# SudeepDasari/visual_foresight

Measured on AMD Instinct MI355X. Metric: predicted frames/sec (whole node), 200-sample x 13-step x 64x64 CEM, higher is better.
Workload: dtype f32

## Files before the change

### visual_foresight_amd/csrc/vf_conv_first.h

```cpp
#pragma once
#include <hip/hip_runtime.h>
#include "vf_conv_mfma.h"

namespace vf {

constexpr int kFirstK = 5, kFirstStride = 2, kFirstCin = 3;
__host__ __device__ constexpr int first_patch_stride(const int TW) { return (((TW - 1) * kFirstStride + kFirstK) * kFirstCin + 1) & ~1; }
__host__ __device__ constexpr size_t first_lds_floats(const int TH, const int TW) {
    return (size_t)((TH - 1) * kFirstStride + kFirstK) * first_patch_stride(TW) + 32;
}

template <int CO, class PT>
__device__ __forceinline__ void conv_first_tile(const PT &p, const int bx_, float *smem) {
    static_assert(CO % 4 == 0 && CO <= 32, "first conv: 4 - 32 output channels");
    typedef const __attribute__((address_space(4))) float cfloat;
    const int bx = __builtin_amdgcn_readfirstlane(bx_);
    const int tid = threadIdx.x, lane = tid & 63, wave = tid >> 6;
    const int tiles_per_img = p.tilesY * p.tilesX;
    const int b = bx / tiles_per_img, tile_id = bx - b * tiles_per_img;
    const int ty0 = (tile_id / p.tilesX) * p.TH, tx0 = (tile_id % p.tilesX) * p.TW;
    const int PH = (p.TH - 1) * kFirstStride + kFirstK, PW3 = ((p.TW - 1) * kFirstStride + kFirstK) * kFirstCin;
    const int PS = first_patch_stride(p.TW);
    float *s_in = smem;
    long long *red = reinterpret_cast<long long *>(smem + (size_t)PH * PS);
// ... 88 lines not shown
            else __builtin_amdgcn_raw_buffer_store_b128(__builtin_bit_cast(u32x4_, v), r_out, o, 0, 0);
        }
        const long long wsum = wave_sum(ssum), wsq = wave_sum(ssq);
        if (lane == 0) { red[2 * wave] = wsum; red[2 * wave + 1] = wsq; }
        __syncthreads();
        if (tid == 0) {
            long long su = 0, sq = 0;
            for (int w = 0; w < 4; ++w) { su += red[2 * w]; sq += red[2 * w + 1]; }
            long long *dst = p.stats + ((long long)b * p.stats_nparts + tile_id) * 2;
            if (wt) {
                __hip_atomic_store(dst, su, __ATOMIC_RELAXED, __HIP_MEMORY_SCOPE_AGENT);
                __hip_atomic_store(dst + 1, sq, __ATOMIC_RELAXED, __HIP_MEMORY_SCOPE_AGENT);
            } else {
                dst[0] = su; dst[1] = sq;
            }
        }
    }
}

template <int CO>
VF_GLOBAL VF_LAUNCH_BOUNDS(kConvThreads, 2) void conv_first_kernel(const ConvParams p) {
    extern __shared__ __attribute__((aligned(16))) float smem[];
    conv_first_tile<CO>(p, blockIdx.x, smem);
}

}
```

### visual_foresight_amd/csrc/vf_conv_mfma.h

```cpp
#pragma once
#include <hip/hip_runtime.h>
#include <type_traits>

#ifdef VF_HOST_SELFTEST
#define VF_GLOBAL __device__
#define VF_LAUNCH_BOUNDS(...)
#else
#define VF_GLOBAL __global__
#define VF_LAUNCH_BOUNDS(...) __launch_bounds__(__VA_ARGS__)
#endif

namespace vf {

constexpr int kPollSleep = 16;

#ifdef VF_TILE_STATS
__device__ unsigned long long g_tile_clk[32][8];
#define VF_TS_NOW() (threadIdx.x == 0 ? wall_clock64() : 0ull)
#define VF_TS_ADD(KEY_, SLOT_, DT_) do { if (threadIdx.x == 0) atomicAdd(&g_tile_clk[KEY_][SLOT_], (unsigned long long)(DT_)); } while (0)
#else
#define VF_TS_NOW() 0ull
#define VF_TS_ADD(KEY_, SLOT_, DT_) do { } while (0)
#endif

// ... 63 lines not shown
__host__ __device__ constexpr int fused_epi(int nd, bool first, bool k6 = false) {
    return EPI_CONVT_FUSED + 2 * (nd - 1) + (first ? 1 : 0) + (k6 ? 8 : 0);
}
__host__ __device__ constexpr int fused_epi_flow(int nd) { return EPI_CONVT_FUSED + 16 + 2 * (nd - 1); }
__host__ __device__ constexpr int fused_epi_dna(int nd) { return fused_epi_flow(nd) + 1; }
static_assert(fused_epi_dna(4) < EPI_CONV_PAIR, "the fused epilogues end in front of EPI_CONV_PAIR");

struct ConvSeg {
    const float *ptr;
    long long bstride;
    int C;
    int nchunk;
    const long long *ln_part;
    long long ln_bstride;
    int ln_nparts;
    float ln_inv_n;
    const float *gamma;
    const float *beta;
    int gamma_mod;
    int relu;
};

struct ConvParams {
    ConvSeg seg[2];
    int nseg;
    int B;
    int Hin, Win;
    int Hout, Wout;
    int KH, KW, stride, pad;
    int KC;
    int NI, TH, TW, RPI;
    int tilesY, tilesX;
    int ncg;
    int Cout;
    const float *Wp;
    const unsigned short *Wp16;
    const float *bias;
    const float *sbias;
    int sbias_ld;
    float *out;
    float *cstate;
    const float *cstate_in;
    long long cin_bstride;
    long long *stats;
    int stats_nparts;
    int chunks_per_split;
    int n_valid;
    int tile_variant;
    const void *fuse_comp;
    const void *fuse_next;
    int *fuse_ready;
    const int *fuse_status;
    int fuse_view, fuse_nd;
    const int *late_cnt;
    int late_expect, late_mode;
    int *late_status;
    int *cu_state;
    int yield_budget;
    int wt_out;
    const float *cond_bias;
// ... 120 lines not shown
        s += __builtin_trunc(d * kStatScale);
        q += __builtin_trunc(d * d * kStatScale);
    }
    __device__ __forceinline__ long long sum() const { return (long long)s; }
    __device__ __forceinline__ long long sumsq() const { return (long long)q; }
};
__device__ __forceinline__ void ln_from_totals(const long long su, const long long sq, const float inv_n,
                                               float &mean, float &rstd) {
    const double m = (double)su * (1.0 / kStatScale) * (double)inv_n;
    double var = (double)sq * (1.0 / kStatScale) * (double)inv_n - m * m;
    var = var < 0.0 ? 0.0 : var;
    mean = (float)m;
    rstd = (float)(1.0 / sqrt(var + (double)kLnEps));
}

struct TileDiv {
    unsigned magic; int d;
    __device__ __forceinline__ explicit TileDiv(const int d_) : magic(0xFFFFFFFFu / (unsigned)d_ + 1u), d(d_) {}
    __device__ __forceinline__ int div(const int n) const { return d == 1 ? n : (int)__umulhi((unsigned)n, magic); }
};

template <class PT>
__device__ __forceinline__ void ln_table(const PT &p, const int bimg0, float *lnTab, const int s_begin = 0,
                                         const int s_end = 2) {
    const int tid = threadIdx.x, lane = tid & 63, wave = tid >> 6;
    const int n = min(s_end, p.nseg) * p.NI, i0 = s_begin * p.NI;
    if (p.nseg * p.NI <= 8) {
        for (int i = i0 + wave; i < n; i += kConvThreads / 64) {
            const int s = i / p.NI, img = i - s * p.NI;
            const auto &sg = p.seg[s];
            float mean = 0.f, rstd = 1.f;
            const int b = bimg0 + img;
            if (sg.ln_part && b < p.B) {
                long long su = 0, sq = 0;
                const long long *pp = sg.ln_part + (long long)b * sg.ln_bstride;
                for (int k = lane; k < sg.ln_nparts; k += 64) { su += pp[2 * k]; sq += pp[2 * k + 1]; }
                su = wave_sum(su); sq = wave_sum(sq);
                ln_from_totals(su, sq, sg.ln_inv_n, mean, rstd);
            }
            if (lane == 0) { lnTab[2 * i] = mean; lnTab[2 * i + 1] = rstd; }
        }
    } else {
        for (int i = i0 + tid; i < n; i += kConvThreads) {
            const int s = i / p.NI, img = i % p.NI;
            const auto &sg = p.seg[s];
            float mean = 0.f, rstd = 1.f;
            const int b = bimg0 + img;
            if (sg.ln_part && b < p.B) {
                long long su = 0, sq = 0;
                const long long *pp = sg.ln_part + (long long)b * sg.ln_bstride;
                for (int k = 0; k < sg.ln_nparts; ++k) { su += pp[2 * k]; sq += pp[2 * k + 1]; }
                ln_from_totals(su, sq, sg.ln_inv_n, mean, rstd);
            }
            lnTab[2 * i] = mean;
            lnTab[2 * i + 1] = rstd;
        }
    }
}

__device__ __forceinline__ void lstm_cell(const float gi, const float gj, const float gf, const float go,
                                          const float c_old, float &c_new, float &h_new) {
    c_new = fmaf(c_old, sigmoidf_(gf + 1.0f), sigmoidf_(gi) * tanhf_(gj));
    h_new = tanhf_(c_new) * sigmoidf_(go);
}

struct LstmRowAddr {
// ... 214 lines not shown
        if (lane == 0) { red[2 * wave] = wsum; red[2 * wave + 1] = wsq; }
        __syncthreads();
        auto put = [&](long long *dst, const long long su, const long long sq) {
            if (p.wt_out != 0) {
                __hip_atomic_store(dst, su, __ATOMIC_RELAXED, __HIP_MEMORY_SCOPE_AGENT);
                __hip_atomic_store(dst + 1, sq, __ATOMIC_RELAXED, __HIP_MEMORY_SCOPE_AGENT);
            } else {
                dst[0] = su; dst[1] = sq;
            }
        };
        if (p.NI == 1) {
            if (tid == 0 && bimg0 < p.B) {
                long long su = 0, sq = 0;
                for (int w = 0; w < 4; ++w) { su += red[2 * w]; sq += red[2 * w + 1]; }
                put(p.stats + ((long long)bimg0 * p.stats_nparts + tile_id * p.ncg + cg) * 2, su, sq);
            }
        } else {
            const int waves_per_img = p.RPI / WROWS;
            if (lane == 0 && (wave % waves_per_img) == 0) {
                const int img = wave / waves_per_img;
                const int b = bimg0 + img;
                if (img < p.NI && b < p.B) {
                    long long su = 0, sq = 0;
                    for (int w = 0; w < waves_per_img; ++w) { su += red[2 * (wave + w)]; sq += red[2 * (wave + w) + 1]; }
                    put(p.stats + ((long long)b * p.stats_nparts + cg) * 2, su, sq);
                }
            }
        }
    }
}

template <class F, int... I>
__device__ __forceinline__ void static_for_impl(F &&f, std::integer_sequence<int, I...>) {
    (f(std::integral_constant<int, I>{}), ...);
}
template <int N, class F>
__device__ __forceinline__ void static_for(F &&f) { static_for_impl(f, std::make_integer_sequence<int, N>{}); }

template <int MR, class PT>
__device__ __forceinline__ void gs_acc_init(const PT &p, f32x16 (&acc)[MR][1], const int cg, const int ty0, const int tx0) {
// ... 158 lines not shown
        for (int img = 0; img < p.NI; ++img) {
            if (bimg0 + img >= p.B) continue;
            long long su = 0, sq = 0;
            for (int w = 0; w < 4; ++w) {
                const int wrb = MR < 4 ? (w & (MR - 1)) : w;
                if (p.NI == 1 || (wrb * 32) / p.RPI == img) { su += red[2 * w]; sq += red[2 * w + 1]; }
            }
            long long *dst = p.stats + ((long long)(bimg0 + img) * p.stats_nparts +
                                        (p.NI == 1 ? tile_id * p.ncg + cg : cg)) * 2;
            if (wt) {
                __hip_atomic_store(dst, su, __ATOMIC_RELAXED, __HIP_MEMORY_SCOPE_AGENT);
                __hip_atomic_store(dst + 1, sq, __ATOMIC_RELAXED, __HIP_MEMORY_SCOPE_AGENT);
            } else {
                dst[0] = su; dst[1] = sq;
            }
        }
    }
}

template <int MR, class PT>
__device__ __forceinline__ void gates_raw_epilogue(const PT &p, f32x16 (&acc)[MR][1], const int bx, const int by, float *smem) {
    static_assert(MR == 4, "raw gate epilogue: 128-row tile");
    const int tid = threadIdx.x, lane = tid & 63, wave = tid >> 6;
    const int cg = by;
    const int tiles_per_img = p.tilesY * p.tilesX;
    int bimg0, ty0, tx0;
    if (p.NI == 1) {
        bimg0 = bx / tiles_per_img;
        const int tile_id = bx % tiles_per_img;
        ty0 = (tile_id / p.tilesX) * p.TH;
// ... 813 lines not shown
```

### visual_foresight_amd/csrc/vf_engine.hip

```cpp
#include <hip/hip_runtime.h>

#include <algorithm>
#include <cmath>
#include <cstdio>
#include <cstring>
#include <cstdlib>
#include <string>
#include <type_traits>
#include <vector>

#include <dlfcn.h>
#ifdef VF_HOST_SELFTEST
#include <sys/mman.h>
#endif

#include "../../include/vf_hip.h"
#include "vf_conv_mfma.h"
#include "vf_small_kernels.h"
#include "vf_goal_image.h"
#include "vf_frame_scorer.h"
#include "vf_registration_net.h"
#include "vf_inverse_model.h"
#include "vf_plan_render.h"
#include "vf_resize.h"
// ... 492 lines not shown
    } sched[2];
    int last_sched = 0;
    size_t sched_capacity = 0, counter_capacity = 0;
    PhaseDesc *stage[kSchedRing] = {nullptr};
    hipEvent_t stage_done[kSchedRing] = {nullptr};
    bool stage_used[kSchedRing] = {false};
    int stage_next = 0;
    int *d_sync = nullptr;
    int xcd_queues = kQueues;
    bool early_start = true;
    bool fuse_top = true;
    bool fuse_pair = true;
    bool wt_publish = VF_WT_DEFAULT != 0;
    bool pad_skip = true;
    bool share_recurrent = true;
    int yield_budget = -1;
    bool pair_allowed = true;
    int *d_status = nullptr;
    unsigned long long *d_stats = nullptr;
    bool phase_stats = false;
    int persist_wgs_per_cu = 2;
    size_t max_lds = 0;

    bool cache_shared = true, shared_valid = false;
    int shared_cfg = -1;

    bool profiling = false;
    std::vector<hipEvent_t> ev_pool;
    size_t ev_used = 0;
    double prof_flops = 0.0;
// ... 432 lines not shown
    }
    VF_ALLOC(h->ctx_states, (size_t)nc * c.sdim);
    VF_ALLOC(h->ctx_actions, (size_t)std::max(nc - 1, 1) * c.adim);

    row_spec(h, h->base.frames_all, (size_t)T * H * W * 3, false);
    if (ND > 0) row_spec(h, h->base.distrib_all, (size_t)T * H * W * ND, false);
    row_spec(h, h->base.states_all, (size_t)T * c.sdim, false);
    if ((rc = alloc_view(h, h->base, (size_t)Bc * NV, false))) return rc;
    h->frames_all = h->base.frames_all; h->distrib_all = h->base.distrib_all; h->states_all = h->base.states_all;
    h->sums_view_stride = (long long)Bc * ND * h->nblocks * 2;
    h->sums_step_stride = h->sums_view_stride * NV;
    if (ND > 0) VF_ALLOC(h->sums, (size_t)T * h->sums_step_stride);
    VF_ALLOC(h->goal_mse, (size_t)Bc * NV * T);
    VF_ALLOC(h->actions_buf, (size_t)Bc * T * c.adim);
    h->sched_capacity = ((size_t)h->S * phases_per_step + 8) * NV;
    h->counter_capacity = h->sched_capacity * ((size_t)Bc + 1);
    VF_ALLOC(h->sched[0].d_phases, h->sched_capacity);
    VF_ALLOC(h->sched[1].d_phases, h->sched_capacity);
    VF_ALLOC(h->d_sync, kSyncHead + h->counter_capacity);
    VF_ALLOC(h->d_status, 1);
    VF_ALLOC(h->d_stats, h->sched_capacity * 2);
    return VF_OK;
}

#define VF_EMIT(var, expr)                 \
    const int var = (expr);                \
    if (Sink::failed(var)) return var;

#include "vf_engine_savp3.inc"

extern "C" {

int vf_abi_version(void) { return VF_ABI_VERSION; }

// ... 210 lines not shown
int vf_create(const vf_config *cfg, vf_handle **out) {
    vf_handle *made = nullptr;
    VF_API_TRY
    if (!out) return fail(VF_ERR_INVALID, "null out pointer");
    *out = nullptr;
    int rc = validate(cfg);
    if (rc) return rc;
#ifndef VF_HOST_SELFTEST
    VF_HIP_CHECK(hipSetDevice(cfg->device));
#endif
    vf_handle *h = new vf_handle();
    made = h;
    h->cfg = *cfg;
    if (const char *e = getenv("VF_PAD_SKIP")) h->pad_skip = atoi(e) != 0;
    if (const char *e = getenv("VF_SHARE_RECURRENT")) h->share_recurrent = atoi(e) != 0;
    h->ncam = std::max(1, cfg->ncam);
    h->n_draws = std::max(1, cfg->n_draws);
    h->cfg.ncam = h->ncam; h->cfg.n_draws = h->n_draws;
    h->H = cfg->height; h->W = cfg->width; h->ND = cfg->ndesig; h->K = cfg->num_masks;
    h->T = cfg->sequence_length - cfg->n_context;
    h->S = h->T + cfg->n_context - 1;
    h->table = tensor_table(*cfg);
    h->blob_floats = h->table.back().offset + h->table.back().size();
    h->savp = cfg->arch == 1 || cfg->arch == 2;
    h->cond = cfg->arch == 2;
    h->flow = is_flow(*cfg);
    h->dna = is_dna(*cfg);
    h->stp = is_stp(*cfg);
    h->Hc = h->savp ? h->H / 2 : h->H; h->Wc = h->savp ? h->W / 2 : h->W;
    const int H = h->H, W = h->W;
// ... 345 lines not shown
            int , int dfin, bool ) {
        int rc = conv(PH_CONVT_RAW, l, p, {});
        if (rc) return rc;
        return composite(cp, ntiles, view, {dfin});
    }
    static bool failed(int rc) { return rc != VF_OK; }
};
#endif

struct ScheduleSink {
    std::vector<PhaseDesc> phases;
    int next_ticket = 0, next_counter = 0;
    double flops = 0.0;
    size_t max_lds = 0;

    static PhaseDep dep_on(const PhaseDesc &Q) {
        PhaseDep dp;
        dp.cnt_base = Q.cnt_base;
        if (Q.whole) { dp.mode = 1; dp.expect = Q.n_items; }
        else {
            dp.mode = (Q.B == 1) ? 1 : 0;
            switch (Q.type) {
                case PH_SA: case PH_CDNA_FIN: case PH_COND: case PH_STP_FIN: dp.expect = 1; break;
                case PH_COMPOSITE: dp.expect = Q.gx; break;
                case PH_EW: dp.expect = Q.ew.spi > 0 ? 1 : Q.gx; break;
                default: dp.expect = (Q.NI == 1 ? Q.tiles_per_img : 1) * Q.gy;
            }
        }
        return dp;
    }
// ... 34 lines not shown
        P.ew = p; P.view = view;
        P.gx = p.spi > 0 ? 1 : p.gx; P.gy = 1;
        max_lds = std::max(max_lds, ew_lds_bytes(p.op, p.op == EW_TOP3 ? p.top.ND : 1));
        return add(P, ew_items(p), p.B, deps);
    }
    int conv_late(int type, const ConvLayer &l, const ConvParams &p, int u_early, int u_late, int u_extra = -1) {
        PhaseDep ld;
        if (!late_dep(u_late, ld)) return conv(type, l, p, {u_early, u_late, u_extra});
        const int u = conv(type, l, p, {u_early, u_extra});
        if (u >= 0) { phases[u].has_late = 1; phases[u].late = ld; }
        return u;
    }
    int conv(int type, const ConvLayer &l, const ConvParams &p, std::initializer_list<int> deps) {
        PhaseDesc P = phase(type, p.B);
        P.conv = p;
        P.NI = l.NI; P.tiles_per_img = l.tilesY * l.tilesX;
        P.gx = conv_items_x(l, p.B);
        P.gy = l.ncg;
        if (l.tile == TILE_FC_WIDE) P.gy = 1;
        P.whole = type == PH_FC_PARTIAL;
        P.tile = l.tile; P.mrep = l.mrep;
        P.prec = p.tile_variant;
        max_lds = std::max(max_lds, l.lds_bytes);
        flops += conv_flops(type, l, p);
        return add(P, P.gx * P.gy * l.nsplit, P.whole ? 1 : p.B, deps);
    }
    int sa(const SaParams &p, std::initializer_list<int> deps) {
        PhaseDesc P = phase(PH_SA, p.B);
        P.sa = p;
        return add(P, (p.B + kSaPerItem - 1) / kSaPerItem, p.B, deps);
    }
    static bool pair_capable() { return true; }
    static const ConvLayer &fc_plan(const vf_handle *h) { return h->fc_wide_ok ? h->fc_wide : h->fc; }
    static bool pairable(const ConvLayer &a, const ConvLayer &b) {
        return a.mode == PACK_PLAIN && b.mode == PACK_PLAIN && a.nseg == 1 && b.nseg == 1 && a.ncg == 2 && b.ncg == 2 &&
               a.Cout == 64 && b.segC[0] == 64 && b.Cout <= 64 && b.KH == 1 && b.KW == 1 && b.stride == 1 && b.pad == 0 &&
               b.KC == 32 && a.tilesY * a.tilesX == 1 && b.tilesY * b.tilesX == 1 && a.NI == b.NI && a.RPI == b.RPI &&
               a.TH == b.TH && a.TW == b.TW && a.Hout == b.Hout && a.Wout == b.Wout && a.nsplit == 1 && b.nsplit == 1 &&
               (a.KH * a.KW * (a.KC / 8)) % 2 == 0 &&
               a.lds_bytes >= (size_t)2 * 128 * 36 * 4;
    }
    int conv_pair(const ConvLayer &a, const ConvParams &pa, const ConvLayer &b, const ConvParams &pb,
                  std::initializer_list<int> deps) {
        PhaseDesc P = phase(PH_CONV_PAIR, pa.B);
        P.conv = pa; P.conv2 = pb;
        P.conv.ncg = 1;
        P.NI = a.NI; P.tiles_per_img = 1;
        P.gx = (pa.B + a.NI - 1) / a.NI; P.gy = 1;
        P.mrep = 1;
        max_lds = std::max(max_lds, a.lds_bytes);
        const double rows = (double)pa.B * a.Hout * a.Wout;
        flops += 2.0 * rows * a.KH * a.KW * a.segC[0] * a.Cout + 2.0 * rows * b.segC[0] * b.Cout;
        return add(P, P.gx, pa.B, deps);
    }
    int fin(const FinParams &p, std::initializer_list<int> deps) {
        PhaseDesc P = phase(PH_CDNA_FIN, p.B);
        P.fin = p;
        return add(P, p.B, p.B, deps);
    }
    int stp_fin(const StpFinParams &p, std::initializer_list<int> deps) {
// ... 5 lines not shown
    int composite(const CompositeParams &p, int ntiles, int view, std::initializer_list<int> deps) {
        PhaseDesc P = phase(PH_COMPOSITE, p.B);
        P.comp = p; P.gx = ntiles; P.view = view;
        return add(P, ntiles * p.B, p.B, deps);
    }
    static bool fusable(const ConvLayer &l, int ND) { return top_fusable(l, ND); }
    int top(const ConvLayer &l, const ConvParams &p, const CompositeParams &cp, int ntiles, int view, int d_early,
            int d_late, int dfin, bool fuse) {
        if (!fuse || !fusable(l, cp.ND)) {
            const int u = conv_late(PH_CONVT_RAW, l, p, d_early, d_late);
            if (u < 0) return u;
            return composite(cp, ntiles, view, {u, dfin});
        }
        PhaseDesc P = phase(PH_TOP_FUSED, p.B);
        P.conv = p; P.comp = cp; P.view = view;
        P.NI = 1; P.tiles_per_img = l.tilesY * l.tilesX;
        P.gx = p.B * P.tiles_per_img; P.gy = 1;
        P.mrep = 1;
        P.aux_base = next_counter + p.B;
        max_lds = std::max(max_lds, std::max(l.lds_bytes, fused_top_lds_floats(l.TH, l.TW, cp.ND) * 4));
        flops += 2.0 * (double)p.B * l.Hout * l.Wout * 9.0 * (l.segC[0] + (l.nseg > 1 ? l.segC[1] : 0)) * l.Cout;
        if (!late_dep(d_late, P.late)) return add(P, P.gx, 2 * p.B, {d_early, d_late, dfin});
        P.has_late = 1;
        return add(P, P.gx, 2 * p.B, {d_early, dfin});
    }
    static bool failed(int rc) { return rc < 0; }
    static int skipped() { return kSkipped; }
};

template <class Sink>
// ... 316 lines not shown
    int items = 0, counters = 0;
    int nq = 1, total_q[kQueues] = {0};
    double flops = 0.0;
    size_t lds = 0;
};

static int build_schedule(vf_handle *h, int B, bool skip_shared, BuiltSchedule &out) {
    std::vector<ScheduleSink> sinks(h->ncam);
    VF_INJECT(1);
    int counters = 0, rc;
    out.flops = 0.0;
    size_t max_lds = 0;
    for (int v = 0; v < h->ncam; ++v) {
        sinks[v].next_counter = counters;
        sinks[v].early_start = h->early_start;
        if (h->cfg.arch == 3)
            rc = emit_rollout_s3(h, v, B, h->actions_buf, nullptr, sinks[v]);
        else
            rc = emit_rollout(h, v, make_view(h, v, h->actions_buf), h->shared_views[(size_t)v], B, nullptr, sinks[v],
                              skip_shared);
        if (rc < 0) return rc;
        counters = sinks[v].next_counter;
        out.flops += sinks[v].flops;
        max_lds = std::max(max_lds, sinks[v].max_lds);
    }
    out.phases.clear();
    const size_t n = sinks[0].phases.size();
    for (size_t i = 0; i < n; ++i)
        for (int v = 0; v < h->ncam; ++v) out.phases.push_back(sinks[v].phases[i]);
    int ticket = 0;
// ... 114 lines not shown
    for (const AllocRec &a : h->allocs) {
        const char *lo = static_cast<const char *>(a.p);
        if (q >= lo && q + bytes <= lo + a.bytes) return true;
    }
    return false;
}

extern "C" int vf_selftest_schedule(vf_handle *h, int32_t B, int32_t skip_shared, int64_t *out_items,
                                    uint64_t *out_upload_checksum) {
    VF_API_TRY
    if (!h) return fail(VF_ERR_INVALID, "null handle");
    BuiltSchedule bs;
    int rc = build_schedule(h, B, skip_shared != 0, bs);
    if (rc) return rc;
    int ticket = 0;
    for (size_t i = 0; i < bs.phases.size(); ++i) {
        const PhaseDesc &P = bs.phases[i];
        if (P.first_ticket != ticket || P.n_items <= 0) return fail(VF_ERR_INVALID, "tickets are not contiguous");
        ticket += P.n_items;
        if (P.ndep < 0 || P.ndep > kMaxDeps) return fail(VF_ERR_INVALID, "bad dependency count");
        if ((h->flow || h->dna) && (P.type == PH_FC_PARTIAL || P.type == PH_CDNA_FIN))
            return fail(VF_ERR_INVALID, "phase " + std::to_string(i) + ": a CDNA kernel item in " +
                                        (h->dna ? "a DNA schedule" : "an appearance-flow schedule"));
        if (h->stp ? P.type == PH_CDNA_FIN : P.type == PH_STP_FIN)
            return fail(VF_ERR_INVALID, "phase " + std::to_string(i) + (h->stp ? ": a CDNA kernel-finish item (a 5 x 5 kernel table) in an STP schedule"
                                                                              : ": an STP finish item outside an STP schedule"));
        for (int d = 0; d < P.ndep; ++d) {
            bool found = false;
            for (size_t j = 0; j < i && !found; ++j) found = bs.phases[j].cnt_base == P.dep[d].cnt_base;
            if (!found) return fail(VF_ERR_INVALID, "phase " + std::to_string(i) + " depends on a later phase");
// ... 12 lines not shown
            const ConvParams &c2 = P.conv2;
            ok = ok && P.conv.ncg == 1 && c2.ncg == 2 && c2.KC == 32 && c2.nseg == 1 && c2.seg[0].nchunk == 2;
            ok = ok && in_allocs(h, c2.Wp, (size_t)2 * 4 * 2 * 64 * 4 * 4) && in_allocs(h, c2.bias, 64 * 4);
            ok = ok && in_allocs(h, c2.out, (size_t)P.B * c2.Hout * c2.Wout * c2.Cout * 4);
            ok = ok && in_allocs(h, c2.sbias, c2.sbias ? (size_t)((P.B - 1) * c2.sbias_ld + c2.Cout) * 4 : 0);
        }
        if (P.type <= PH_FC_PARTIAL || ph_is_conv(P.type) || P.type == PH_TOP_FUSED || P.type == PH_CONV_PAIR) {
            const ConvParams &c = P.conv;
            for (int s = 0; s < c.nseg; ++s) {
                const long long span = (long long)(P.B - 1) * c.seg[s].bstride + (long long)c.Hin * c.Win * c.seg[s].C;
                ok = ok && in_allocs(h, c.seg[s].ptr, (size_t)span * 4);
                ok = ok && in_allocs(h, c.seg[s].ln_part, c.seg[s].ln_part ? (size_t)((P.B - 1) * c.seg[s].ln_bstride + c.seg[s].ln_nparts * 2) * 8 : 0);
            }
            ok = ok && in_allocs(h, c.Wp, 16) && in_allocs(h, c.bias, 4) && in_allocs(h, c.out, 4);
            ok = ok && in_allocs(h, c.cstate, 4) && in_allocs(h, c.cstate_in, 4) && in_allocs(h, c.stats, 8);
            const size_t gates_bytes = (size_t)c.Hout * c.Wout * 4 * c.Cout * 4;
            if (P.type == PH_GATES_RAW) ok = ok && in_allocs(h, c.out, (size_t)P.B * gates_bytes);
            if (c.chunk_begin != 0)
                ok = ok && (P.type == PH_GATES_RAW ||
                            (P.type == PH_LSTM && (P.tile == TILE_LSTM_GS128 || P.tile == TILE_LSTM_GS64)));
            if (c.acc_init)
                ok = ok && in_allocs(h, c.acc_init, gates_bytes) && P.type == PH_LSTM && P.NI == 1 && !P.has_late &&
                     (P.tile == TILE_LSTM_GS128 || P.tile == TILE_LSTM_GS64) && c.chunk_begin == c.seg[0].nchunk;
        }
        if (P.conv.wt_out != 0) {
            const bool lstm_vec = P.type == PH_LSTM &&
                                  (P.tile == TILE_LSTM_GS128 || P.tile == TILE_LSTM_GS64 || P.tile == TILE_LSTM_ROW32);
            const bool light_vec = P.type >= PH_CONV_RELU && P.type <= PH_CONVT_RAW && P.conv.Cout % 4 == 0 &&
                                   ((P.tile == TILE_CONV && P.mrep == 1) ||
                                    (P.tile == TILE_FIRST_VALU && P.type == PH_CONV_RAW && (P.conv.Cout == 16 || P.conv.Cout == 32)));
// ... 148 lines not shown
                head[q] += P.n_q[q];
                total += P.n_q[q];
            }
            if (bs.nq > 1 && P.q_inner > 1 && ph_is_conv(P.type)) {
                int lo = P.n_q[0], hi = P.n_q[0];
                for (int q = 0; q < bs.nq; ++q) { lo = std::min(lo, P.n_q[q]); hi = std::max(hi, P.n_q[q]); }
                if (hi - lo > 1) return fail(VF_ERR_INVALID, "phase " + std::to_string(i) + ": queues are not balanced");
            }
            for (int q = bs.nq; q < kQueues; ++q)
                if (P.n_q[q]) return fail(VF_ERR_INVALID, "items in an unused queue");
        }
        for (int q = 0; q < bs.nq; ++q)
            if (head[q] != bs.total_q[q]) return fail(VF_ERR_INVALID, "queue totals mismatch");
        if (total != bs.items) return fail(VF_ERR_INVALID, "dealt item count mismatch");
    }
    if (out_items) *out_items = bs.items;
    if (out_upload_checksum) *out_upload_checksum = h->upload_checksum;
    return VF_OK;
    VF_API_CATCH(int)
}
extern "C" int vf_selftest_inject(int32_t where, int32_t kind) {
    g_inject_where = where; g_inject_kind = kind;
    return VF_OK;
}
extern "C" int vf_set_fuse_top(vf_handle *h, int32_t enable) {
    VF_API_TRY
    if (!h) return fail(VF_ERR_INVALID, "null handle");
    h->fuse_top = enable != 0;
    h->fuse_pair = enable != 0;
    return VF_OK;
// ... 150 lines not shown
        sc_host.types.clear(); sc_host.nitems.clear();
        for (const PhaseDesc &P : bs.phases) {
            sc_host.types.push_back(P.type == PH_EW ? 100 + P.ew.op : P.type);
            sc_host.nitems.push_back(P.n_items);
        }
        sc_host.flops = bs.flops;
        sc_host.lds = bs.lds;
    }
    h->last_sched = skip_shared ? 1 : 0;
    if (h->cfg.arch == 3) {
        if ((rc = s3_zero_state(h, B, st))) return rc;
    } else if (!skip_shared)
        for (int v = 0; v < h->ncam; ++v)
            if ((rc = zero_shared_state(h, h->shared_views[(size_t)v], st))) return rc;
    VF_HIP_CHECK(hipMemsetAsync(h->d_sync, 0, (kSyncHead + (size_t)sc_host.counters) * sizeof(int), st));
    Schedule sc;
    memset(&sc, 0, sizeof(sc));
    sc.phases = sc_host.d_phases; sc.n_phases = sc_host.phases; sc.total_items = sc_host.items;
    sc.ticket = h->d_sync; sc.counters = h->d_sync + kSyncHead; sc.status = h->d_status;
    sc.nq = sc_host.nq;
    for (int q = 0; q < kQueues; ++q) sc.total_q[q] = sc_host.total_q[q];
    sc.cu_tab = yield_for(h, B) > 0 ? h->d_sync + kTicketInts : nullptr;
    sc.stats = nullptr;
    sc.nd = h->ND;
    for (int i = 0; i < h->ncam * h->ND * 2; ++i) sc.goal[i] = goal_pix[i];
    if (h->phase_stats) {
        VF_HIP_CHECK(hipMemsetAsync(h->d_stats, 0, h->sched_capacity * 2 * sizeof(unsigned long long), st));
        sc.stats = h->d_stats;
    }

// ... 579 lines not shown
```

### visual_foresight_amd/csrc/vf_fc_tile.h

```cpp
#pragma once
#include <hip/hip_runtime.h>
#include "vf_conv_mfma.h"

namespace vf {

constexpr int kFcRows = 128;
constexpr int kFcGroups = 8;
__host__ __device__ inline size_t fc_wide_lds_bytes() { return (size_t)(kFcRows * 36 + 2 * kFcRows) * 4 + 64; }

template <class PT>
__device__ __forceinline__ void fc_wide_tile(const PT &p, const int bx_, const int bz_, float *smem) {
    const int bx = __builtin_amdgcn_readfirstlane(bx_), bz = __builtin_amdgcn_readfirstlane(bz_);
    constexpr int KCpad = 36, G = kFcGroups;
    const int tid = threadIdx.x, lane = tid & 63, wave = tid >> 6;
    const int n = lane & 31, kh = lane >> 5;
    float *lnTab = smem + kFcRows * KCpad;
    const auto &sg = p.seg[0];
    const int b0 = bx * kFcRows;
    const int n_here = min(kFcRows, p.B - b0);

    if (tid < kFcRows) {
        float mean = 0.f, rstd = 1.f;
        if (sg.ln_part && tid < n_here) {
            long long su = 0, sq = 0;
            const long long *pp = sg.ln_part + (long long)(b0 + tid) * sg.ln_bstride;
            for (int k = 0; k < sg.ln_nparts; ++k) { su += pp[2 * k]; sq += pp[2 * k + 1]; }
            ln_from_totals(su, sq, sg.ln_inv_n, mean, rstd);
        }
        lnTab[2 * tid] = mean; lnTab[2 * tid + 1] = rstd;
    }

    f32x16 acc[G];
#pragma unroll
    for (int g = 0; g < G; ++g)
#pragma unroll
        for (int r = 0; r < 16; ++r) acc[g][r] = 0.f;

    const int ncg = p.ncg;
    const int Ntot = ncg * 32;
    const unsigned w_loff = (unsigned)(((kh * Ntot + n) * 4) * 4);
    const unsigned wstep_b = (unsigned)(2 * Ntot * 4) * 4u;
// ... 84 lines not shown
```

### visual_foresight_amd/csrc/vf_fused_top.h

```cpp
#pragma once
#include <hip/hip_runtime.h>
#include "vf_conv_mfma.h"
#include "vf_small_kernels.h"

namespace vf {

constexpr unsigned kFusedSpinLimit = 1u << 24;
constexpr int kFusedCtlGoal = 8;

__host__ __device__ inline size_t fused_top_lds_floats(int TH, int TW, int ND) {
    const size_t halo = (size_t)(2 * TH + 4) * (2 * TW + 4);
    return (size_t)256 * kCompEncPad + halo * comp_px_stride(ND) + (size_t)kTaps * kCompKernPad + 16 + 64;
}

template <int ND, bool FIRST, int K, class PT, class CT, int MODE = COMP_CDNA>
__device__ __forceinline__ void fused_top_body(const PT &p, const CT &c, f32x16 (&acc)[1][4], const int bx,
                                               long long *red, float *smem, const int *goal) {
    constexpr bool FLOW = MODE == COMP_FLOW, DNA = MODE == COMP_DNA, STP = MODE == COMP_STP, GATHER = FLOW || STP;
    const int tid = threadIdx.x, lane = tid & 63, wave = tid >> 6;
    const int n = lane & 31, kh = lane >> 5;
    const int tiles_per_img = p.tilesY * p.tilesX;
    const int b = bx / tiles_per_img, tile_id = bx - b * tiles_per_img;
    const int ty0 = (tile_id / p.tilesX) * p.TH, tx0 = (tile_id % p.tilesX) * p.TW;
    const TileDiv div_tw(p.TW);
// ... 30 lines not shown
        for (int r = 0; r < 16; ++r)
#pragma unroll
            for (int g = 0; g < 4; ++g)
                if ((okmask >> r) & 1u) { ssum += stat_q(acc[0][g][r]); ssq += stat_q2(acc[0][g][r]); }
    }
    const long long wsum = wave_sum(ssum), wsq = wave_sum(ssq);
    __syncthreads();
    if (lane == 0) { red[2 * wave] = wsum; red[2 * wave + 1] = wsq; }
    __syncthreads();
    if (tid == 0) {
        long long su = 0, sq = 0;
        for (int w = 0; w < 4; ++w) { su += red[2 * w]; sq += red[2 * w + 1]; }
        long long *dst = p.stats + ((long long)b * p.stats_nparts + tile_id) * 2;
        __hip_atomic_store(dst, su, __ATOMIC_RELAXED, __HIP_MEMORY_SCOPE_AGENT);
        __hip_atomic_store(dst + 1, sq, __ATOMIC_RELAXED, __HIP_MEMORY_SCOPE_AGENT);
        asm volatile("s_waitcnt vmcnt(0)" ::: "memory");
        __hip_atomic_fetch_add(p.fuse_ready + b, 1, __ATOMIC_RELAXED, __HIP_MEMORY_SCOPE_AGENT);
    }
    __syncthreads();
    [[maybe_unused]] const unsigned long long tf1 = VF_TS_NOW();
    VF_TRACE_EVT(TR_TOP_STATS);

    const int RH = 2 * p.TH, RW = 2 * p.TW;
    const int HW_ = RW + 4, HH_ = RH + 4;
    const int oy0 = 2 * ty0, ox0 = 2 * tx0;
    float *s_enc = smem;
    constexpr int PS = comp_px_stride(ND);
    float *s_px = s_enc + 256 * kCompEncPad;
    float *s_kern = s_px + HH_ * HW_ * PS;
    float *s_ln = s_kern + kTaps * kCompKernPad;
// ... 85 lines not shown
        unsigned spins = 0;
        int ok = 1;
        if (lane == 0) {
            while (__hip_atomic_load(p.fuse_ready + b, __ATOMIC_RELAXED, __HIP_MEMORY_SCOPE_AGENT) < tiles_per_img) {
                __builtin_amdgcn_s_sleep(8);
                if (++spins > kFusedSpinLimit ||
                    __hip_atomic_load(p.fuse_status, __ATOMIC_RELAXED, __HIP_MEMORY_SCOPE_AGENT) != 0) { ok = 0; break; }
            }
            VF_ACQUIRE_AGENT();
            *s_flag = ok;
        }
        __builtin_amdgcn_wave_barrier();
        ok = __shfl(ok, 0, 64);
        if (ok) {
            long long su = 0, sq = 0;
            const long long *pp = p.stats + (long long)b * p.stats_nparts * 2;
            for (int k = lane; k < tiles_per_img; k += 64) {
                su += __hip_atomic_load(pp + 2 * k, __ATOMIC_RELAXED, __HIP_MEMORY_SCOPE_AGENT);
                sq += __hip_atomic_load(pp + 2 * k + 1, __ATOMIC_RELAXED, __HIP_MEMORY_SCOPE_AGENT);
            }
            su = wave_sum(su); sq = wave_sum(sq);
            if (lane == 0) ln_from_totals(su, sq, c.ln_inv_n, s_ln[0], s_ln[1]);
        }
    }
    __syncthreads();
    if (*s_flag == 0) {
        if (tid == 0) {
            extern __shared__ __attribute__((aligned(16))) float smem_all[];
            atomicExch(const_cast<int *>(p.fuse_status), 1);
            reinterpret_cast<int *>(smem_all)[1] = 0;
        }
        return;
    }
    const float mean = s_ln[0], rstd = s_ln[1];
    [[maybe_unused]] const unsigned long long tf3 = VF_TS_NOW();
    VF_TRACE_EVT(TR_TOP_MATES);
// ... 116 lines not shown
```

Before: 44400.

## Accumulate LayerNorm stat totals atomically at producers instead of re-reducing partials

```diff
diff --git a/visual_foresight_amd/csrc/vf_conv_first.h b/visual_foresight_amd/csrc/vf_conv_first.h
--- a/visual_foresight_amd/csrc/vf_conv_first.h
+++ b/visual_foresight_amd/csrc/vf_conv_first.h
@@ -126,6 +126,7 @@
             } else {
                 dst[0] = su; dst[1] = sq;
             }
+            stat_total_add(p.tot, b, su, sq);
         }
     }
 }
diff --git a/visual_foresight_amd/csrc/vf_conv_mfma.h b/visual_foresight_amd/csrc/vf_conv_mfma.h
--- a/visual_foresight_amd/csrc/vf_conv_mfma.h
+++ b/visual_foresight_amd/csrc/vf_conv_mfma.h
@@ -101,6 +101,7 @@
     const long long *ln_part;
     long long ln_bstride;
     int ln_nparts;
+    const long long *ln_tot;
     float ln_inv_n;
     const float *gamma;
     const float *beta;
@@ -131,6 +132,7 @@
     long long cin_bstride;
     long long *stats;
     int stats_nparts;
+    long long *tot;
     int chunks_per_split;
     int n_valid;
     int tile_variant;
@@ -281,6 +283,16 @@
     rstd = (float)(1.0 / sqrt(var + (double)kLnEps));
 }
 
+__device__ __forceinline__ void stat_total_add(long long *tot, const int b, const long long su, const long long sq) {
+    if (tot == nullptr) return;
+    __hip_atomic_fetch_add(tot + 2 * (long long)b, su, __ATOMIC_RELAXED, __HIP_MEMORY_SCOPE_AGENT);
+    __hip_atomic_fetch_add(tot + 2 * (long long)b + 1, sq, __ATOMIC_RELAXED, __HIP_MEMORY_SCOPE_AGENT);
+}
+__device__ __forceinline__ void stat_total_load(const long long *slot, long long &su, long long &sq) {
+    su = __hip_atomic_load(slot, __ATOMIC_RELAXED, __HIP_MEMORY_SCOPE_AGENT);
+    sq = __hip_atomic_load(slot + 1, __ATOMIC_RELAXED, __HIP_MEMORY_SCOPE_AGENT);
+}
+
 struct TileDiv {
     unsigned magic; int d;
     __device__ __forceinline__ explicit TileDiv(const int d_) : magic(0xFFFFFFFFu / (unsigned)d_ + 1u), d(d_) {}
@@ -300,9 +312,13 @@
             const int b = bimg0 + img;
             if (sg.ln_part && b < p.B) {
                 long long su = 0, sq = 0;
-                const long long *pp = sg.ln_part + (long long)b * sg.ln_bstride;
-                for (int k = lane; k < sg.ln_nparts; k += 64) { su += pp[2 * k]; sq += pp[2 * k + 1]; }
-                su = wave_sum(su); sq = wave_sum(sq);
+                if (sg.ln_tot) {
+                    stat_total_load(sg.ln_tot + (sg.ln_bstride ? 2 * (long long)b : 0), su, sq);
+                } else {
+                    const long long *pp = sg.ln_part + (long long)b * sg.ln_bstride;
+                    for (int k = lane; k < sg.ln_nparts; k += 64) { su += pp[2 * k]; sq += pp[2 * k + 1]; }
+                    su = wave_sum(su); sq = wave_sum(sq);
+                }
                 ln_from_totals(su, sq, sg.ln_inv_n, mean, rstd);
             }
             if (lane == 0) { lnTab[2 * i] = mean; lnTab[2 * i + 1] = rstd; }
@@ -315,8 +331,12 @@
             const int b = bimg0 + img;
             if (sg.ln_part && b < p.B) {
                 long long su = 0, sq = 0;
-                const long long *pp = sg.ln_part + (long long)b * sg.ln_bstride;
-                for (int k = 0; k < sg.ln_nparts; ++k) { su += pp[2 * k]; sq += pp[2 * k + 1]; }
+                if (sg.ln_tot) {
+                    stat_total_load(sg.ln_tot + (sg.ln_bstride ? 2 * (long long)b : 0), su, sq);
+                } else {
+                    const long long *pp = sg.ln_part + (long long)b * sg.ln_bstride;
+                    for (int k = 0; k < sg.ln_nparts; ++k) { su += pp[2 * k]; sq += pp[2 * k + 1]; }
+                }
                 ln_from_totals(su, sq, sg.ln_inv_n, mean, rstd);
             }
             lnTab[2 * i] = mean;
@@ -561,6 +581,7 @@
                 long long su = 0, sq = 0;
                 for (int w = 0; w < 4; ++w) { su += red[2 * w]; sq += red[2 * w + 1]; }
                 put(p.stats + ((long long)bimg0 * p.stats_nparts + tile_id * p.ncg + cg) * 2, su, sq);
+                stat_total_add(p.tot, bimg0, su, sq);
             }
         } else {
             const int waves_per_img = p.RPI / WROWS;
@@ -571,6 +592,7 @@
                     long long su = 0, sq = 0;
                     for (int w = 0; w < waves_per_img; ++w) { su += red[2 * (wave + w)]; sq += red[2 * (wave + w) + 1]; }
                     put(p.stats + ((long long)b * p.stats_nparts + cg) * 2, su, sq);
+                    stat_total_add(p.tot, b, su, sq);
                 }
             }
         }
@@ -759,6 +781,7 @@
             } else {
                 dst[0] = su; dst[1] = sq;
             }
+            stat_total_add(p.tot, bimg0 + img, su, sq);
         }
     }
 }
diff --git a/visual_foresight_amd/csrc/vf_engine.hip b/visual_foresight_amd/csrc/vf_engine.hip
--- a/visual_foresight_amd/csrc/vf_engine.hip
+++ b/visual_foresight_amd/csrc/vf_engine.hip
@@ -5,6 +5,7 @@
 #include <cstdio>
 #include <cstring>
 #include <cstdlib>
+#include <map>
 #include <string>
 #include <type_traits>
 #include <vector>
@@ -530,6 +531,10 @@
     bool wt_publish = VF_WT_DEFAULT != 0;
     bool pad_skip = true;
     bool share_recurrent = true;
+    bool ln_totals = true;
+    long long *d_sh_tot = nullptr;
+    int sh_tot_slots = 0;
+    std::vector<std::map<const long long *, const long long *>> sh_tot_last;
     int yield_budget = -1;
     bool pair_allowed = true;
     int *d_status = nullptr;
@@ -992,10 +997,13 @@
     VF_ALLOC(h->goal_mse, (size_t)Bc * NV * T);
     VF_ALLOC(h->actions_buf, (size_t)Bc * T * c.adim);
     h->sched_capacity = ((size_t)h->S * phases_per_step + 8) * NV;
-    h->counter_capacity = h->sched_capacity * ((size_t)Bc + 1);
+    h->counter_capacity = h->sched_capacity * ((size_t)Bc * 6 + 4);
     VF_ALLOC(h->sched[0].d_phases, h->sched_capacity);
     VF_ALLOC(h->sched[1].d_phases, h->sched_capacity);
     VF_ALLOC(h->d_sync, kSyncHead + h->counter_capacity);
+    h->sh_tot_slots = h->S * kNumLn;
+    VF_ALLOC(h->d_sh_tot, (size_t)NV * h->sh_tot_slots * 2);
+    h->sh_tot_last.assign((size_t)NV, {});
     VF_ALLOC(h->d_status, 1);
     VF_ALLOC(h->d_stats, h->sched_capacity * 2);
     return VF_OK;
@@ -1236,6 +1244,7 @@
     h->cfg = *cfg;
     if (const char *e = getenv("VF_PAD_SKIP")) h->pad_skip = atoi(e) != 0;
     if (const char *e = getenv("VF_SHARE_RECURRENT")) h->share_recurrent = atoi(e) != 0;
+    if (const char *e = getenv("VF_LN_TOTALS")) h->ln_totals = atoi(e) != 0;
     h->ncam = std::max(1, cfg->ncam);
     h->n_draws = std::max(1, cfg->n_draws);
     h->cfg.ncam = h->ncam; h->cfg.n_draws = h->n_draws;
@@ -1611,6 +1620,36 @@
     double flops = 0.0;
     size_t max_lds = 0;
 
+    int *counter0 = nullptr;
+    long long *sh_tot = nullptr;
+    int sh_tot_n = 0, sh_tot_next = 0;
+    std::vector<const long long *> sh_stats;
+    std::map<const long long *, const long long *> tot_of;
+    std::map<const long long *, const long long *> *sh_last = nullptr;
+    int link_totals(ConvParams &c) {
+        if (!counter0) return VF_OK;
+        for (int s = 0; s < c.nseg; ++s) {
+            ConvSeg &sg = c.seg[s];
+            sg.ln_tot = nullptr;
+            if (!sg.ln_part) continue;
+            auto it = tot_of.find(sg.ln_part);
+            if (it != tot_of.end()) sg.ln_tot = it->second;
+            else if (sg.ln_bstride == 0 && sh_last && sh_last->count(sg.ln_part)) sg.ln_tot = sh_last->at(sg.ln_part);
+        }
+        if (!c.stats) return VF_OK;
+        if (std::find(sh_stats.begin(), sh_stats.end(), c.stats) != sh_stats.end()) {
+            if (c.B != 1 || sh_tot_next >= sh_tot_n) return fail(VF_ERR_INVALID, "shared LayerNorm totals: out of slots");
+            c.tot = sh_tot + 2 * (size_t)sh_tot_next++;
+            if (sh_last) (*sh_last)[c.stats] = c.tot;
+        } else {
+            next_counter = (next_counter + 3) & ~3;
+            c.tot = reinterpret_cast<long long *>(counter0 + next_counter);
+            next_counter += 4 * c.B;
+        }
+        tot_of[c.stats] = c.tot;
+        return VF_OK;
+    }
+
     static PhaseDep dep_on(const PhaseDesc &Q) {
         PhaseDep dp;
         dp.cnt_base = Q.cnt_base;
@@ -1675,6 +1714,7 @@
     int conv(int type, const ConvLayer &l, const ConvParams &p, std::initializer_list<int> deps) {
         PhaseDesc P = phase(type, p.B);
         P.conv = p;
+        if (int rc = link_totals(P.conv)) return rc;
         P.NI = l.NI; P.tiles_per_img = l.tilesY * l.tilesX;
         P.gx = conv_items_x(l, p.B);
         P.gy = l.ncg;
@@ -1705,6 +1745,8 @@
                   std::initializer_list<int> deps) {
         PhaseDesc P = phase(PH_CONV_PAIR, pa.B);
         P.conv = pa; P.conv2 = pb;
+        if (pa.stats || pb.stats || pb.seg[0].ln_part) return fail(VF_ERR_INVALID, "conv pair: neither conv writes LayerNorm partials, the second reads none");
+        if (int rc = link_totals(P.conv)) return rc;
         P.conv.ncg = 1;
         P.NI = a.NI; P.tiles_per_img = 1;
         P.gx = (pa.B + a.NI - 1) / a.NI; P.gy = 1;
@@ -1740,6 +1782,7 @@
         }
         PhaseDesc P = phase(PH_TOP_FUSED, p.B);
         P.conv = p; P.comp = cp; P.view = view;
+        if (int rc = link_totals(P.conv)) return rc;
         P.NI = 1; P.tiles_per_img = l.tilesY * l.tilesX;
         P.gx = p.B * P.tiles_per_img; P.gy = 1;
         P.mrep = 1;
@@ -2086,6 +2129,19 @@
     for (int v = 0; v < h->ncam; ++v) {
         sinks[v].next_counter = counters;
         sinks[v].early_start = h->early_start;
+        if (h->ln_totals && h->cfg.arch != 3) {
+            static_assert(kSyncHead % 4 == 0, "the totals' slots are 16-byte aligned behind the head of d_sync");
+            const BatchView &sv = h->shared_views[(size_t)v];
+            sinks[v].counter0 = h->d_sync + kSyncHead;
+            sinks[v].sh_tot = h->d_sh_tot + (size_t)v * h->sh_tot_slots * 2;
+            sinks[v].sh_tot_n = h->sh_tot_slots;
+            sinks[v].sh_stats = {sv.st_enc00, sv.st_enc0, sv.st_h[0], sv.st_h[1], sv.st_h[2], sv.st_h[3], sv.st_h[4],
+                                 sv.st_h[5], sv.st_h[6]};
+            sinks[v].sh_stats.erase(std::remove(sinks[v].sh_stats.begin(), sinks[v].sh_stats.end(), nullptr),
+                                    sinks[v].sh_stats.end());
+            if (!skip_shared) h->sh_tot_last[(size_t)v].clear();
+            sinks[v].sh_last = &h->sh_tot_last[(size_t)v];
+        }
         if (h->cfg.arch == 3)
             rc = emit_rollout_s3(h, v, B, h->actions_buf, nullptr, sinks[v]);
         else
@@ -2230,6 +2286,7 @@
     int rc = build_schedule(h, B, skip_shared != 0, bs);
     if (rc) return rc;
     int ticket = 0;
+    int n_tot_prod = 0, n_tot_shared = 0, n_tot_linked = 0, n_tot_cached = 0, n_tot_reduce = 0;
     for (size_t i = 0; i < bs.phases.size(); ++i) {
         const PhaseDesc &P = bs.phases[i];
         if (P.first_ticket != ticket || P.n_items <= 0) return fail(VF_ERR_INVALID, "tickets are not contiguous");
@@ -2272,6 +2329,57 @@
             }
             ok = ok && in_allocs(h, c.Wp, 16) && in_allocs(h, c.bias, 4) && in_allocs(h, c.out, 4);
             ok = ok && in_allocs(h, c.cstate, 4) && in_allocs(h, c.cstate_in, 4) && in_allocs(h, c.stats, 8);
+            const bool want_tot = h->ln_totals && h->cfg.arch != 3;
+            const char *cnt_lo = reinterpret_cast<const char *>(h->d_sync + kSyncHead);
+            const char *sh_lo = reinterpret_cast<const char *>(h->d_sh_tot);
+            const char *sh_hi = sh_lo + (size_t)h->ncam * h->sh_tot_slots * 16;
+            auto in_shared = [&](const void *q) {
+                const char *a = static_cast<const char *>(q);
+                return a >= sh_lo && a + 16 <= sh_hi && (a - sh_lo) % 16 == 0;
+            };
+            if ((c.tot != nullptr) != (want_tot && c.stats != nullptr)) return fail(VF_ERR_INVALID, "phase " + std::to_string(i) + ": LayerNorm totals slot where none belongs, or none where one does");
+            if (c.tot) {
+                const char *a = reinterpret_cast<const char *>(c.tot);
+                const bool sh_unit = std::any_of(h->shared_views.begin(), h->shared_views.end(), [&](const BatchView &sv) {
+                    bool m = c.stats == sv.st_enc00 || c.stats == sv.st_enc0;
+                    for (int k = 0; k < 7; ++k) m = m || c.stats == sv.st_h[k];
+                    return m;
+                });
+                if (sh_unit) {
+                    if (P.B != 1 || !in_shared(c.tot) || skip_shared) return fail(VF_ERR_INVALID, "phase " + std::to_string(i) + ": bad shared totals slot");
+                    ++n_tot_shared;
+                } else {
+                    const long long off = a - cnt_lo;
+                    if (off < 0 || off % 16 || off + 16LL * P.B != 4LL * P.cnt_base)
+                        return fail(VF_ERR_INVALID, "phase " + std::to_string(i) + ": totals slot not directly in front of the phase's counters");
+                }
+                for (size_t j = 0; j < i; ++j)
+                    if (bs.phases[j].conv.tot == c.tot)
+                        return fail(VF_ERR_INVALID, "phase " + std::to_string(i) + ": totals slot used twice");
+                ++n_tot_prod;
+            }
+            for (int s = 0; s < c.nseg; ++s) {
+                const ConvSeg &sg = c.seg[s];
+                if (!sg.ln_part) {
+                    if (sg.ln_tot) return fail(VF_ERR_INVALID, "phase " + std::to_string(i) + ": totals without partials");
+                    continue;
+                }
+                const PhaseDesc *prod = nullptr;
+                for (size_t j = 0; j < i; ++j)
+                    if (bs.phases[j].conv.stats == sg.ln_part) prod = &bs.phases[j];
+                if (prod) {
+                    if (sg.ln_tot != prod->conv.tot)
+                        return fail(VF_ERR_INVALID, "phase " + std::to_string(i) + " segment " + std::to_string(s) + ": totals of another phase than the producer of its partials");
+                    if (sg.ln_bstride == 0 ? prod->B != 1 : prod->B != P.B)
+                        return fail(VF_ERR_INVALID, "phase " + std::to_string(i) + " segment " + std::to_string(s) + ": producer of another batch size");
+                    n_tot_linked += sg.ln_tot ? 1 : 0;
+                } else {
+                    if (!skip_shared || sg.ln_bstride != 0 || (sg.ln_tot && !in_shared(sg.ln_tot)))
+                        return fail(VF_ERR_INVALID, "phase " + std::to_string(i) + " segment " + std::to_string(s) + ": partials nobody in this schedule writes");
+                    n_tot_cached += sg.ln_tot ? 1 : 0;
+                }
+                if (!sg.ln_tot) ++n_tot_reduce;
+            }
             const size_t gates_bytes = (size_t)c.Hout * c.Wout * 4 * c.Cout * 4;
             if (P.type == PH_GATES_RAW) ok = ok && in_allocs(h, c.out, (size_t)P.B * gates_bytes);
             if (c.chunk_begin != 0)
@@ -2450,6 +2558,10 @@
             if (head[q] != bs.total_q[q]) return fail(VF_ERR_INVALID, "queue totals mismatch");
         if (total != bs.items) return fail(VF_ERR_INVALID, "dealt item count mismatch");
     }
+    if (getenv("VF_SELFTEST_LN_TOTALS"))
+        std::printf("    ln-totals B=%d %s: %d producer phases (%d shared), segments: %d linked, %d on cached shared slots, %d reducing partials; "
+                    "%d of %d ints cleared per launch\n", (int)B, skip_shared ? "cached-context" : "full", n_tot_prod, n_tot_shared,
+                    n_tot_linked, n_tot_cached, n_tot_reduce, kSyncHead + bs.counters, (int)(kSyncHead + h->counter_capacity));
     if (out_items) *out_items = bs.items;
     if (out_upload_checksum) *out_upload_checksum = h->upload_checksum;
     return VF_OK;
@@ -2630,6 +2742,8 @@
         for (int v = 0; v < h->ncam; ++v)
             if ((rc = zero_shared_state(h, h->shared_views[(size_t)v], st))) return rc;
     VF_HIP_CHECK(hipMemsetAsync(h->d_sync, 0, (kSyncHead + (size_t)sc_host.counters) * sizeof(int), st));
+    if (!skip_shared && h->ln_totals)
+        VF_HIP_CHECK(hipMemsetAsync(h->d_sh_tot, 0, (size_t)h->ncam * h->sh_tot_slots * 2 * sizeof(long long), st));
     Schedule sc;
     memset(&sc, 0, sizeof(sc));
     sc.phases = sc_host.d_phases; sc.n_phases = sc_host.phases; sc.total_items = sc_host.items;
diff --git a/visual_foresight_amd/csrc/vf_fc_tile.h b/visual_foresight_amd/csrc/vf_fc_tile.h
--- a/visual_foresight_amd/csrc/vf_fc_tile.h
+++ b/visual_foresight_amd/csrc/vf_fc_tile.h
@@ -23,8 +23,12 @@
         float mean = 0.f, rstd = 1.f;
         if (sg.ln_part && tid < n_here) {
             long long su = 0, sq = 0;
-            const long long *pp = sg.ln_part + (long long)(b0 + tid) * sg.ln_bstride;
-            for (int k = 0; k < sg.ln_nparts; ++k) { su += pp[2 * k]; sq += pp[2 * k + 1]; }
+            if (sg.ln_tot) {
+                stat_total_load(sg.ln_tot + (sg.ln_bstride ? 2 * (long long)(b0 + tid) : 0), su, sq);
+            } else {
+                const long long *pp = sg.ln_part + (long long)(b0 + tid) * sg.ln_bstride;
+                for (int k = 0; k < sg.ln_nparts; ++k) { su += pp[2 * k]; sq += pp[2 * k + 1]; }
+            }
             ln_from_totals(su, sq, sg.ln_inv_n, mean, rstd);
         }
         lnTab[2 * tid] = mean; lnTab[2 * tid + 1] = rstd;
diff --git a/visual_foresight_amd/csrc/vf_fused_top.h b/visual_foresight_amd/csrc/vf_fused_top.h
--- a/visual_foresight_amd/csrc/vf_fused_top.h
+++ b/visual_foresight_amd/csrc/vf_fused_top.h
@@ -68,6 +68,7 @@
         long long *dst = p.stats + ((long long)b * p.stats_nparts + tile_id) * 2;
         __hip_atomic_store(dst, su, __ATOMIC_RELAXED, __HIP_MEMORY_SCOPE_AGENT);
         __hip_atomic_store(dst + 1, sq, __ATOMIC_RELAXED, __HIP_MEMORY_SCOPE_AGENT);
+        stat_total_add(p.tot, b, su, sq);
         asm volatile("s_waitcnt vmcnt(0)" ::: "memory");
         __hip_atomic_fetch_add(p.fuse_ready + b, 1, __ATOMIC_RELAXED, __HIP_MEMORY_SCOPE_AGENT);
     }
@@ -183,12 +184,16 @@
         ok = __shfl(ok, 0, 64);
         if (ok) {
             long long su = 0, sq = 0;
-            const long long *pp = p.stats + (long long)b * p.stats_nparts * 2;
-            for (int k = lane; k < tiles_per_img; k += 64) {
-                su += __hip_atomic_load(pp + 2 * k, __ATOMIC_RELAXED, __HIP_MEMORY_SCOPE_AGENT);
-                sq += __hip_atomic_load(pp + 2 * k + 1, __ATOMIC_RELAXED, __HIP_MEMORY_SCOPE_AGENT);
-            }
-            su = wave_sum(su); sq = wave_sum(sq);
+            if (p.tot) {
+                stat_total_load(p.tot + 2 * (long long)b, su, sq);
+            } else {
+                const long long *pp = p.stats + (long long)b * p.stats_nparts * 2;
+                for (int k = lane; k < tiles_per_img; k += 64) {
+                    su += __hip_atomic_load(pp + 2 * k, __ATOMIC_RELAXED, __HIP_MEMORY_SCOPE_AGENT);
+                    sq += __hip_atomic_load(pp + 2 * k + 1, __ATOMIC_RELAXED, __HIP_MEMORY_SCOPE_AGENT);
+                }
+                su = wave_sum(su); sq = wave_sum(sq);
+            }
             if (lane == 0) ln_from_totals(su, sq, c.ln_inv_n, s_ln[0], s_ln[1]);
         }
     }
```

New measurement: 44410, median of 2. No clear change (+0.0%).
